# author-hidden-name/GAN-segmentation

Hardware: AMD Instinct MI355X
Metric: synthetic (image,mask) pairs/sec, FFHQ-1024 StyleGAN+decoder (higher is better)
Workload: dtype f32; 1 GPU; stylegan-ffhq 1024^2 synthesis + 2-class decoder, batch=8 per GPU, fp32 (BASELINE.json configs[1]); synthetic weights/latents/noise; (img u8, mask u8) resident on rank 0; global_batch=8, parallelism=dp1, gather=none, backend=none, graph=eager (GSA_GRAPH=0)

## Files before the change

### gan-segmentation_amd/csrc/gsa_api.cpp

```cpp
#include <hip/hip_runtime.h>

#include <cmath>
#include <cstdarg>
#include <cstdio>
#include <cstdlib>
#include <cstring>
#include <map>
#include <string>
#include <vector>

#include "../../include/gsa.h"
#include "gsa_kernels.h"
#include "gsa_pack.h"

using namespace gsa;

namespace {

constexpr int kMaxLevels = 12;
thread_local std::string g_create_error;

struct HostTensor {
    std::vector<float> data;
    std::vector<int64_t> dims;
// ... 780 lines not shown
                              uint8_t* img, float* const* feats, bool record_levels) {
    const int L = c->gc.latent_size, nlev = c->nlev;
    const double N = n;
    if (z) {
        if (int rc = run_mapping(c, s, n, z, c->lat[0])) return rc;
        const float* w = c->lat[0];
        Launch lp(c, s, "g.styles", 2.0 * N * L * c->style_cols, 4.0 * ((double)L * c->style_cols + N * c->style_cols));
        HIP_TRY(launch_styles(w, c->latent_avg, c->psi, c->style_wt, c->style_b, c->style_col_layer, c->styles, n, L, c->style_cols, s));
    } else {
        Launch lp(c, s, "g.styles", 2.0 * N * L * c->style_cols, 4.0 * ((double)L * c->style_cols + N * 2 * nlev * L + N * c->style_cols));
        HIP_TRY(launch_styles_dlatents(dl, c->latent_avg, c->psi, c->style_wt, c->style_b, c->style_tiles, c->style_num_tiles, c->styles, n, L,
                                       c->style_cols, 2 * nlev, s));
    }

    char layer[64];
    for (int l = 0; l < nlev; ++l) {
        const GenBlockDev& B = c->blk[l];
        const int R = B.R, C = B.C, Cin = B.Cin;
        const double px = N * R * R;
        for (int k = 0; k < 2; ++k) {
            const float* nz = noise[2 * l + k];
            if (!nz) return fail(c, GSA_ERR_INVALID, "noise plane %d is null", 2 * l + k);
            int prow = 0;
            if (k == 0) {
                PostParams pp{};
                pp.noise = nz; pp.nscale = B.nscale[0]; pp.nbias = B.nbias[0];
                pp.out = c->x1; pp.partials = c->partials; pp.H = R; pp.W = R; pp.C = C; pp.bf16 = c->bf16;
                if (!B.has_conv1) {
                    pp.src = c->constant; pp.src_per_sample = 0; pp.blur = nullptr;
                } else {
                    ConvParams cp = conv_base(c);
                    cp.src0 = c->x2[l - 1]; cp.aff0 = c->aff2[l - 1]; cp.C0 = Cin;
                    cp.Hs = R / 2; cp.Ws = R / 2; cp.H = R; cp.W = R;
                    cp.wpk = B.w1; cp.Cout = C; cp.out = c->t_raw;
                    if (B.is_deconv || R >= 16) {
                        snprintf(layer, sizeof layer, B.is_deconv ? "g.%d.deconv_1" : "g.%d.conv_1", R);
                        Launch lp(c, s, layer, 2.0 * px * C * Cin * (subpixel_uses_wino(cp) ? 2.25 : 4.0), 4.0 * (px / 4 * Cin + px * C), 2.0 * px * C * Cin * (B.is_deconv ? 4 : 9));
                        HIP_TRY(launch_subpixel(cp, EPI_RAW, false, n, s));
                    } else {
                        cp.up = 1;
                        snprintf(layer, sizeof layer, "g.%d.conv_1", R);
                        Launch lp(c, s, layer, 2.0 * px * C * Cin * 9, 4.0 * (px / 4 * Cin + px * C));
                        HIP_TRY(launch_conv3x3(cp, EPI_RAW, false, n, s));
                    }
                    pp.src = c->t_raw; pp.src_per_sample = 1; pp.blur = B.blur;
                }
                snprintf(layer, sizeof layer, "g.%d.post_1", R);
                if (post_fuses_finalize(pp)) {
                    FinalizeParams fp{};
                    fp.partials = c->partials; fp.prow = 0; fp.HW = R * R; fp.C = C; fp.acc = c->stat_acc; fp.tickets = c->stat_tickets;
                    fp.style = c->styles + B.style_off[0]; fp.style_stride = c->style_cols;
                    fp.gamma = B.gamma[0]; fp.beta = B.beta[0];
                    fp.aff = c->aff1;
                    fp.flags = c->map_ctl;
                    Launch lp(c, s, layer, 0.0, 4.0 * (2 * px * C + px));
                    HIP_TRY(launch_post_fin(pp, fp, n, s));
                    continue;
                }
                Launch lp(c, s, layer, 0.0, 4.0 * (2 * px * C + px));
#ifdef GSA_DBG_HOOKS
                if (!((c->dbg & 8) && R >= 512))
#endif
                HIP_TRY(launch_post(pp, n, s));
                prow = post_rows_used(pp);
            } else {
                ConvParams cp = conv_base(c);
                cp.src0 = c->x1; cp.aff0 = c->aff1; cp.C0 = C;
                cp.Hs = R; cp.Ws = R; cp.H = R; cp.W = R;
                cp.wpk = B.w2; cp.wino = B.w2u; cp.Cout = C; cp.out = c->x2[l];
                cp.noise = nz; cp.nscale = B.nscale[1]; cp.nbias = B.nbias[1]; cp.partials = c->partials;
                snprintf(layer, sizeof layer, "g.%d.conv_2", R);
                int rows = conv_stat_rows(R, R, C, n);
                cp.stat_rows_host = &rows;
                const bool fused_fin = conv_fuses_finalize(cp, EPI_SYNTH, false);
                const double products = conv_form_products(conv3x3_form(cp, EPI_SYNTH, false));
                if (fused_fin) {
                    cp.fin_style = c->styles + B.style_off[1]; cp.fin_style_stride = c->style_cols;
                    cp.fin_gamma = B.gamma[1]; cp.fin_beta = B.beta[1]; cp.fin_aff = c->aff2[l]; cp.fin_flags = c->map_ctl;
                }
                Launch lp(c, s, layer, 2.0 * px * C * C * products, 4.0 * (2 * px * C + px), 2.0 * px * C * C * 9);
                HIP_TRY(launch_conv3x3(cp, EPI_SYNTH, false, n, s));
                prow = rows;
                if (fused_fin) continue;
            }
            if (c->fault == 2 && l == 3 && k == 1) {
                c->fault = 0;
                return fail(c, GSA_ERR_HIP, "injected fault (gsa_debug_inject 2) between a statistics producer and its finalize");
            }
            FinalizeParams fp{};
            fp.partials = c->partials; fp.prow = prow; fp.HW = R * R; fp.C = C; fp.acc = c->stat_acc; fp.tickets = c->stat_tickets;
            fp.style = c->styles + B.style_off[k]; fp.style_stride = c->style_cols;
            fp.gamma = B.gamma[k]; fp.beta = B.beta[k];
            fp.aff = k == 0 ? c->aff1 : c->aff2[l];
            fp.flags = c->map_ctl;
            snprintf(layer, sizeof layer, "g.%d.finalize_%d", R, k + 1);
#ifdef GSA_DBG_HOOKS
            if ((c->dbg & 32) && ((k == 0 && R <= 32) || (k == 1 && R <= 8))) continue;
            if ((c->dbg & 64)) continue;
#endif
            Launch lp(c, s, layer, 0.0, 16.0 * N * prow * C);
            HIP_TRY(launch_finalize(fp, n, s));
        }
        if (record_levels) HIP_TRY(hipEventRecord(c->ev_level[l], s));
        if (feats && feats[l]) {
            snprintf(layer, sizeof layer, "g.%d.export", R);
            Launch lp(c, s, layer, 0.0, 8.0 * px * C);
            HIP_TRY(launch_export_nchw(c->x2[l], c->aff2[l], feats[l], n, R, R, C, c->bf16, s));
        }
    }
    if (rgb || img) {
        const int l = nlev - 1, R = c->blk[l].R, C = c->blk[l].C, nc = c->gc.channels;
// ... 354 lines not shown
```

### gan-segmentation_amd/csrc/gsa_dev.h

```cpp
#pragma once
#include "gsa_kernels.h"

#ifndef GSA_NO_XCD_REMAP
#define GSA_NO_XCD_REMAP 0
#endif

namespace gsa {

#ifdef GSA_STAMP
#define GSA_DBG_HOOKS 1
#endif
#ifdef GSA_STAMP
#define STAMP(i) do { __builtin_amdgcn_sched_barrier(0); asm volatile("s_memtime %0\n\ts_waitcnt lgkmcnt(0)" : "=s"(stamp_t[i]) :: "memory"); __builtin_amdgcn_sched_barrier(0); } while (0)
#define STAMP_DECL unsigned long long stamp_t[8] = {0, 0, 0, 0, 0, 0, 0, 0}
#define STAMP_FLUSH(nph) do { if (p.stamps && (threadIdx.x & 63) == 0) { for (int i_ = 0; i_ < (nph); ++i_) atomicAdd(&p.stamps[i_], stamp_t[i_ + 1] - stamp_t[i_]); atomicAdd(&p.stamps[15], 1ull); } } while (0)
#define TICK(var) do { __builtin_amdgcn_sched_barrier(0); asm volatile("s_memtime %0\n\ts_waitcnt lgkmcnt(0)" : "=s"(var) :: "memory"); __builtin_amdgcn_sched_barrier(0); } while (0)
#define TSUM(acc, a, b) acc += (b) - (a)
#define TFLUSH(idx, acc) do { if (p.stamps && (threadIdx.x & 63) == 0) atomicAdd(&p.stamps[idx], acc); } while (0)
#else
#define TICK(var) do {} while (0)
#define TSUM(acc, a, b) do {} while (0)
#define TFLUSH(idx, acc) do {} while (0)
#define STAMP(i) do {} while (0)
#define STAMP_DECL do {} while (0)
// ... 130 lines not shown

template <bool BF>
__device__ __forceinline__ f32x4 act_load4(const float* base, size_t idx) {
    if constexpr (BF) {
        const u32x2 r = *reinterpret_cast<const u32x2*>(reinterpret_cast<const unsigned short*>(base) + idx);
        return f32x4{bf16_lo(r[0]), bf16_hi(r[0]), bf16_lo(r[1]), bf16_hi(r[1])};
    } else {
        return *reinterpret_cast<const f32x4*>(base + idx);
    }
}

template <bool BF>
__device__ __forceinline__ void act_store4(float* base, size_t idx, const f32x4& v) {
    if constexpr (BF) {
        *reinterpret_cast<u32x2*>(reinterpret_cast<unsigned short*>(base) + idx) =
            u32x2{__builtin_bit_cast(unsigned, __builtin_convertvector(f32x2{v[0], v[1]}, bf16x2)),
                  __builtin_bit_cast(unsigned, __builtin_convertvector(f32x2{v[2], v[3]}, bf16x2))};
    } else {
        *reinterpret_cast<f32x4*>(base + idx) = v;
    }
}


__device__ __forceinline__ int xcd_block(int b, int nb) {
    return (nb & 7) == 0 && !GSA_NO_XCD_REMAP ? (b & 7) * (nb >> 3) + (b >> 3) : b;
}


}
```

### gan-segmentation_amd/csrc/gsa_kernels.h

```cpp
#pragma once
#include <hip/hip_runtime.h>
#include <stdint.h>
#include <stdlib.h>

#include <atomic>
#include <string>

namespace gsa {

struct Aff { float mean, A, B, pad; };

struct StatPart { unsigned long long s1, s2; };

constexpr double kStatScale1 = 268435456.0;

enum Epilogue { EPI_RAW = 0, EPI_SYNTH = 1, EPI_DEC = 2 };

struct ConvParams {
    int device;
    const float* src0; const Aff* aff0; int C0;
    const float* src1; int C1;
    int Hs, Ws;
    int up;
    int H, W;
    const float* wpk;
    const float* wino;
    int Cout;
    float* out;
    const float* noise; const float* nscale; const float* nbias;
    StatPart* partials; int prow;
    const float* bn_s; const float* bn_beta;
    const float* resid; int resid_up;
    const float* resid1; int res_c0;
    const float* wsc; const float* sc_bias; float* out_sc;
    int tiles_x, tiles_y, groups, total_tiles;
    int stats_direct;
    int* stat_rows_host;
    int w_resident;
    int group_minor;
    unsigned long long* stamps;
    int dbg;
    int prio;
    int bf16;
    const float* fin_style; int fin_style_stride; const float* fin_gamma; const float* fin_beta; Aff* fin_aff; unsigned* fin_flags;
    const float* zeros;
    const float* rgb_w; const float* rgb_b; uint8_t* rgb_img;
};

struct PostParams {
    const float* src;
    int src_per_sample;
    const float* blur;
    const float* noise; const float* nscale; const float* nbias;
    float* out; StatPart* partials; int prow;
    int H, W, C;
    int bf16;
    int row_groups;
};

struct FinalizeParams {
    const StatPart* partials; int prow; int HW; int C;
    StatPart* acc;
    unsigned* tickets;
    const float* style; int style_stride;
    const float* gamma; const float* beta;
    Aff* aff;
    unsigned* flags;
};

inline int env_int(const char* name, int dflt) {
    const char* v = getenv(name);
    return v ? atoi(v) : dflt;
}


enum class ConvForm { Wino43, WinoDma, WinoTwoTiles, WinoLean, Wino, KSplit, Bf16Lean, Direct };
ConvForm conv3x3_form(const ConvParams& p, int epi, bool shortcut);
hipError_t launch_conv3x3(const ConvParams& p, int epi, bool shortcut, int n, hipStream_t s);
inline bool conv_form_wino(ConvForm f) { return f <= ConvForm::Wino; }
inline double conv_form_products(ConvForm f) { return f == ConvForm::Wino43 ? 2.25 : conv_form_wino(f) ? 4 : 9; }
// ... 14 lines not shown
    int ct;
    SubPath path;
    bool wino;
    int kb;
    size_t lds;
    int wgs_per_group;
};
SubpixelPlan subpixel_plan(const ConvParams& p, bool shortcut, int n);
hipError_t launch_subpixel(const ConvParams& p, int epi, bool shortcut, int n, hipStream_t s);
bool subpixel_uses_wino(const ConvParams& p);
enum class PostKind { Dma, Packed, Rows, OneRow };
struct PostPlan { PostKind kind; int rpt, row_groups, blocks, rows_used; };
PostPlan post_plan(const PostParams& p);
hipError_t launch_post(const PostParams& p, int n, hipStream_t s);
int post_pk_mode();
bool post_dma_applies(const PostParams& p);
int post_dma_band(const PostParams& p);
int post_dma_blocks(const PostParams& p);
hipError_t launch_post_dma(const PostParams& p, int n, hipStream_t s);
hipError_t launch_post_pk(const PostParams& q, dim3 grid, size_t lds, hipStream_t s);
hipError_t launch_finalize(const FinalizeParams& p, int n, hipStream_t s);
bool conv_fuses_finalize(const ConvParams& p, int epi, bool shortcut);
bool post_fuses_finalize(const PostParams& p);
hipError_t launch_post_fin(const PostParams& p, const FinalizeParams& f, int n, hipStream_t s);
hipError_t launch_pixelnorm(const float* z, float* out, int n, int L, hipStream_t s);
constexpr int kMapSlices = 8;
bool mapping_fused(int L, int device);
hipError_t launch_mapping(const float* z, float* const* wt, float* const* b, unsigned long long* const* ll, float* out, unsigned* ctl,
                          int n, int L, int device, hipStream_t s, int drop_workgroups = 0);
hipError_t launch_dense(const float* x, const float* WT, const float* b, float* y, int n, int K, int J,
                        int lrelu, hipStream_t s);
hipError_t launch_styles(const float* w, const float* avg, const float* psi, const float* WT, const float* b,
                         const int* col_layer, float* styles, int n, int K, int J, hipStream_t s);
hipError_t launch_styles_dlatents(const float* dlatents, const float* avg, const float* psi, const float* WT, const float* b,
                                  const int4* tiles, int num_tiles, float* styles, int n, int K, int J, int NL, hipStream_t s);
hipError_t launch_torgb(const float* x, const Aff* aff, const float* w, const float* b, float* rgb,
                        uint8_t* img, int n, int H, int W, int C, int nc, int bf16, hipStream_t s);
hipError_t launch_torgb_down(const float* x, const Aff* aff, const float* w, const float* b, uint8_t* img, int n, int H, int W, int C,
                             int nc, int f, int bf16, hipStream_t s);
hipError_t launch_final_conv_down(const float* src0, int C0, const float* src1, int C1, const float* wpk, const float* bias, uint8_t* mask,
                                  int n, int H, int W, int ncls, int f, int bf16, hipStream_t s);
hipError_t launch_export_nchw(const float* x, const Aff* aff, float* out, int n, int H, int W, int C, int bf16, hipStream_t s);
hipError_t launch_import_nhwc(const float* in, float* out, int n, int H, int W, int C, int bf16, hipStream_t s);
hipError_t launch_final_conv(const float* src0, int C0, const float* src1, int C1, const float* wpk,
                             const float* bias, float* logits, uint8_t* mask, int n, int H, int W, int ncls, int bf16,
                             hipStream_t s);
// ... 45 lines not shown
```

### gan-segmentation_amd/csrc/gsa_kernels.hip

```cpp
#include "gsa_kernels.h"
#include "gsa_dev.h"

#include <cxxabi.h>

#include <cstdio>
#include <cstdlib>
#include <cstring>
#include <mutex>
#include <vector>

#ifndef GSA_MFMA_PRIO
#define GSA_MFMA_PRIO 2
#endif
#ifndef GSA_OPERAND_PIPELINE
#define GSA_OPERAND_PIPELINE 1
#endif
#ifndef GSA_NO_XCD_REMAP
#define GSA_NO_XCD_REMAP 0
#endif
#ifndef GSA_POST_OCC
#define GSA_POST_OCC 2
#endif
#ifndef GSA_WINO_SOA
#define GSA_WINO_SOA 0
// ... 628 lines not shown
        __syncthreads();
        if (has_aff && tn.n != n_aff) {
            write_aff();
            n_aff = tn.n;
            __syncthreads();
        }
#ifdef GSA_DBG_HOOKS
        if (!(p.dbg & 8))
#endif
        write_item(cb2, tpn, is_edge(tn));
        __syncthreads();
        tc = tn; w = w2; cb = cb2;
#pragma unroll
        for (int it = 0; it < AIT; ++it) tp[it] = tpn[it];
    }
    STAMP(4);
#ifdef GSA_STAMP
    asm volatile("s_waitcnt vmcnt(0)" ::: "memory");
#endif
    STAMP(5);
    STAMP_FLUSH(5);
}

__device__ __forceinline__ void finalize_one(const FinalizeParams& p, int n, int c, unsigned long long I1, unsigned long long I2);
template <int TH, int EPI, bool BF, int PS>
__global__ __launch_bounds__(256 * PS) void conv3x3_ksplit(ConvParams p) {
    constexpr int NTHR = 256 * PS, MT = (TH / 4) * (TH / 4), PW = TH / 4;
    constexpr int MTW = MT / PS;
    constexpr int LH = TH + 2, LW = TH + 2, NPX = LH * LW;
    constexpr int PX = BF ? 8 : 16, TS = BF ? 128 : 256, KQ = BF ? 2 : 4;
    constexpr int RS = LW * PX + (BF ? 4 : 8);
    constexpr int SEG = 9 * TS, IMG = LH * RS;
    constexpr int NB4 = 4 * SEG / 4, BIT = (NB4 + NTHR - 1) / NTHR;
    constexpr int QPT = PS == 1 ? 4 : 1;
    static_assert(PS == 1 || (PS == 2 && MT == 4 && 4 * NPX <= NTHR), "patch split: 8x8 tiles, one staged unit per thread");
    static_assert(NPX <= NTHR, "one staged pixel per thread and block");
    extern __shared__ __attribute__((aligned(16))) float smem[];
    float* sA = smem;
    float* sB = sA + 2 * 4 * IMG;
    f32x4* sAff = reinterpret_cast<f32x4*>(sB + 2 * 4 * SEG);
    f32x4* sP = sAff + 2 * 4 * 16;
    unsigned long long (*sfin)[16] = reinterpret_cast<unsigned long long (*)[16]>(sP + 4 * MT * 64);
    unsigned& sfin_cnt = *reinterpret_cast<unsigned*>(sfin + 2);
    if (EPI == EPI_SYNTH && p.fin_aff != nullptr && threadIdx.x < 33) {
        if (threadIdx.x < 32) sfin[threadIdx.x >> 4][threadIdx.x & 15] = 0ull; else sfin_cnt = 0u;
    }

// ... 1964 lines not shown
            }
        }
#pragma unroll
        for (int j = 0; j < 4; ++j) {
            atomicAdd(&sstat[c + j], I1[j]);
            atomicAdd(&sstat[p.C + c + j], I2[j]);
        }
    }
    __syncthreads();
    if ((int)gridDim.x > p.prow) {
        for (int i = threadIdx.x; i < p.C; i += 256) {
            StatPart* a = p.partials + ((size_t)n * p.prow + (blockIdx.x & (kDirectRows - 1))) * p.C + i;
            atomicAdd(&a->s1, sstat[i]);
            atomicAdd(&a->s2, sstat[p.C + i]);
        }
        return;
    }
    for (int i = threadIdx.x; i < p.C; i += 256) {
        StatPart sp; sp.s1 = sstat[i]; sp.s2 = sstat[p.C + i];
        p.partials[((size_t)n * p.prow + blockIdx.x) * p.C + i] = sp;
    }
}

__device__ __forceinline__ void finalize_one(const FinalizeParams& p, int n, int c, unsigned long long I1, unsigned long long I2) {
    const double inv_hw = 1.0 / (double)p.HW;
    const double m = (double)(long long)I1 * (1.0 / kStatScale1) * inv_hw;
    const double e2 = (double)(long long)I2 * (1.0 / stat_scale2(p.HW)) * inv_hw;
    double var = fma(-m, m, e2);
    {
        const long long s1 = (long long)I1;
        const bool near_wrap = (s1 < 0 ? -s1 : s1) >= (1ll << 61) || I2 >= (1ull << 61);
        if (p.flags && (near_wrap || var < -1e-6 * (e2 + m * m) - 1e-30)) atomicOr(p.flags, 1u);
    }
    if (!(var > 0.0)) var = 0.0;
    const float mean_f = (float)m, var_f = (float)var;
    const float inv = 1.0f / sqrtf(var_f + 1e-5f);
    const float gsc = p.gamma[c] * inv;
    const float* st = p.style + (size_t)n * p.style_stride;
    const float s1 = st[c] + 1.0f;
    Aff a;
    a.mean = mean_f;
    a.A = gsc * s1;
    a.B = fmaf(-mean_f, a.A, fmaf(p.beta[c], s1, st[p.C + c]));
    a.pad = 0.0f;
    p.aff[(size_t)n * p.C + c] = a;
}

__global__ __launch_bounds__(256) void finalize_kernel(FinalizeParams p, int rows_per_block) {
    __shared__ unsigned long long sh[2][256];
    __shared__ int is_last;
    const int n = blockIdx.y;
    const int cblk = p.C >= 64 ? 64 : p.C, nrg = 256 / cblk;
    const int cl = threadIdx.x % cblk, rg = threadIdx.x / cblk;
    const int c = blockIdx.x * 64 + cl;
    unsigned long long I1 = 0, I2 = 0;
    if (rg < nrg && c < p.C) {
        const int r0 = blockIdx.z * rows_per_block;
        const int r1 = min(p.prow, r0 + rows_per_block);
        const StatPart* base = p.partials + (size_t)n * p.prow * p.C + c;
#pragma unroll 16
        for (int r = r0 + rg; r < r1; r += nrg) {
            const StatPart sp = base[(size_t)r * p.C];
            I1 += sp.s1; I2 += sp.s2;
        }
        StatPart zero; zero.s1 = 0ull; zero.s2 = 0ull;
        StatPart* wbase = const_cast<StatPart*>(base);
        for (int r = r0 + rg; r < r1; r += nrg) wbase[(size_t)r * p.C] = zero;
    }
    sh[0][threadIdx.x] = I1; sh[1][threadIdx.x] = I2;
    __syncthreads();
// ... 933 lines not shown
    switch (conv3x3_form(p, epi, sc)) {
#if GSA_EXPERIMENTS
        case ConvForm::Wino43: return launch_wino43(p, epi, n, s);
        case ConvForm::WinoDma: return launch_wino_dma(p, epi, n, s);
        case ConvForm::WinoTwoTiles: return launch_wino_two_tiles(p, epi, n, s);
#endif
        case ConvForm::WinoLean: return launch_wino_lean(p, epi, n, s);
        case ConvForm::Wino: return launch_wino(p, epi, n, s);
        case ConvForm::KSplit: return launch_ksplit(p, epi, n, s);
        case ConvForm::Bf16Lean: return launch_bf16_lean(p, epi, n, s);
        case ConvForm::Direct: return launch_direct(p, epi, sc, n, s);
        default: return hipErrorInvalidValue;
    }
}

static bool fuse_finalize() {
    static const bool enabled = env_int("GSA_FUSEFIN", 1) != 0;
    return enabled;
}
bool conv_fuses_finalize(const ConvParams& p, int epi, bool sc) {
    return fuse_finalize() && epi == EPI_SYNTH && p.H <= 8 && conv3x3_form(p, epi, sc) == ConvForm::KSplit;
}

bool conv_fuses_torgb(const ConvParams& p, int epi, bool sc, int nc) {
    return conv3x3_form(p, epi, sc) == ConvForm::WinoLean && wino_lean_fuses_torgb(p, epi, nc);
}

bool subpixel_uses_wino(const ConvParams& p) {
    static const bool enabled = env_int("GSA_WINO22", 1) != 0;
    return enabled && !p.bf16;
}

SubpixelPlan subpixel_plan(const ConvParams& p, bool sc, int n) {
    static const bool res_enabled = env_int("GSA_SUBRES", 1) != 0;
    static const bool wst_enabled = env_int("GSA_SUBWST", 1) != 0;
    SubpixelPlan plan{};
    plan.wino = subpixel_uses_wino(p);
    const long tiles = (long)(p.H / 16) * (p.W / 16) * n;
    plan.ct = 16;
    for (int ct = plan.wino ? 32 : 64; ct > 16; ct /= 2)
        if (p.Cout % ct == 0 && tiles * (p.Cout / ct) >= 512) { plan.ct = ct; break; }
    const int ts = p.bf16 ? 128 : 256, nt = plan.ct / 16;
    const int rs = p.bf16 ? 10 * 8 + 4 : 10 * 16 + (plan.wino ? 4 : 8);
    if (res_enabled && plan.ct == p.Cout && plan.ct <= 32 && tiles >= 4096) {
        const int nblk = (p.C0 + p.C1) / 16;
        const size_t panel = sizeof(float) * ((size_t)nblk * nt * 16 * ts + (sc ? (size_t)nblk * nt * ts : 0));
// ... 106 lines not shown
    q.prow = plan.rows_used;
    q.row_groups = plan.row_groups;
    const dim3 grid(plan.blocks, n);
    const size_t lds = sizeof(unsigned long long) * 2 * p.C;
    const int dev = current_device();
    switch (plan.kind) {
        case PostKind::Dma: return launch_post_dma(q, n, s);
        case PostKind::Packed: return launch_post_pk(q, grid, lds + sizeof(float) * 9 * p.C, s);
        default: break;
    }
#define GSA_POST(BF) \
    if (plan.rpt == 8) return launch<post_rows_kernel<8, BF>>(dev, grid, dim3(256), lds, s, q); \
    if (plan.rpt == 4) return launch<post_rows_kernel<4, BF>>(dev, grid, dim3(256), lds, s, q); \
    if (plan.rpt == 2) return launch<post_rows_kernel<2, BF>>(dev, grid, dim3(256), lds, s, q); \
    return launch<post_kernel<BF>>(dev, grid, dim3(256), lds, s, q);
    if (p.bf16) { GSA_POST(true) }
    GSA_POST(false)
#undef GSA_POST
}

bool post_fuses_finalize(const PostParams& p) {
    return fuse_finalize() && p.H * p.W <= 1024 && p.C % 16 == 0 && p.W % 4 == 0;
}
hipError_t launch_post_fin(const PostParams& p, const FinalizeParams& f, int n, hipStream_t s) {
    if (!post_fuses_finalize(p)) return hipErrorInvalidValue;
    dim3 grid(p.C / 16, n);
    if (p.bf16) return launch<post_fin_kernel<true>>(current_device(), grid, dim3(256), 0, s, p, f);
    return launch<post_fin_kernel<false>>(current_device(), grid, dim3(256), 0, s, p, f);
}

hipError_t launch_finalize(const FinalizeParams& p, int n, hipStream_t s) {
    const int rpb = std::min(256, std::max(64, (p.prow + 15) / 16));
    const int zb = (p.prow + rpb - 1) / rpb;
    dim3 grid((p.C + 63) / 64, n, zb < 1 ? 1 : zb);
    return launch<finalize_kernel>(current_device(), grid, dim3(256), 0, s, p, rpb);
}

hipError_t launch_pixelnorm(const float* z, float* out, int n, int L, hipStream_t s) {
    return launch<pixelnorm_kernel>(current_device(), dim3(n), dim3(64), sizeof(float) * L, s, z, out, n, L);
}

hipError_t launch_dense(const float* x, const float* WT, const float* b, float* y, int n, int K, int J, int act, hipStream_t s) {
    if (K % 256 || J % 4) return hipErrorInvalidValue;
    const size_t lds = sizeof(float) * (256 * 16 + 16 * 256 + 256);
    return launch<dense_lds_kernel<false, 16, 256>>(current_device(), dim3((J + 15) / 16), dim3(256), lds, s, x, WT, b, y, n, K, J, act,
                  (const float*)nullptr, (const float*)nullptr, (const int*)nullptr);
// ... 112 lines not shown
```

### gan-segmentation_amd/csrc/gsa_post_lean.hip

```cpp
#include "gsa_kernels.h"
#include "gsa_dev.h"

#include <cstdlib>

namespace gsa {
namespace lean {

template <bool NT, bool BF>
__global__ __launch_bounds__(256, 2) void post_rows_pk(PostParams p) {
    constexpr int RPT = 4, ES = BF ? 2 : 4;
    extern __shared__ __attribute__((aligned(16))) unsigned long long sstat[];
    float* const sW = reinterpret_cast<float*>(sstat + 2 * p.C);
    const int n = blockIdx.y;
    const int C4 = p.C >> 2, W4 = p.W >> 2;
    const int NG = p.row_groups > 1 ? p.row_groups : 1;
    const int total = (p.H / (RPT * NG)) * W4 * C4;
    for (int i = threadIdx.x; i < 2 * p.C; i += 256) sstat[i] = 0ull;
    for (int i = threadIdx.x; i < 9 * p.C; i += 256) sW[(i % 9) * p.C + i / 9] = p.blur[i];
    __syncthreads();
    const int idx = xcd_block(blockIdx.x, gridDim.x) * 256 + threadIdx.x;
    if (idx < total) {
        const int cq = idx % C4, t = idx / C4;
        const int xq = t % W4;
        const int y0 = __builtin_amdgcn_readfirstlane((t / W4) * (RPT * NG));
        const int c = cq * 4, x0 = xq * 4;
        const char* const sb = reinterpret_cast<const char*>(p.src) + (size_t)n * p.H * p.W * p.C * ES;
        char* const ob = reinterpret_cast<char*>(p.out) + (size_t)n * p.H * p.W * p.C * ES;
        const char* const nzb = reinterpret_cast<const char*>(p.noise + (size_t)n * p.H * p.W);
        const volatile f32x4* wtap = reinterpret_cast<const volatile f32x4*>(sW + c);
// ... 59 lines not shown
                v01[q] = a; v23[q] = b;
                const f32x4 o = {a.x, a.y, b.x, b.y};
                char* dst = orow + xoff[1 + q];
                if constexpr (BF) act_store4<true>(reinterpret_cast<float*>(dst), 0, o);
                else if (NT) __builtin_nontemporal_store(o, reinterpret_cast<f32x4*>(dst));
                else *reinterpret_cast<f32x4*>(dst) = o;
            }
            const f32x2 s01 = (v01[0] + v01[1]) + (v01[2] + v01[3]);
            const f32x2 s23 = (v23[0] + v23[1]) + (v23[2] + v23[3]);
            const f32x2 q01 = (v01[0] * v01[0] + v01[1] * v01[1]) + (v01[2] * v01[2] + v01[3] * v01[3]);
            const f32x2 q23 = (v23[0] * v23[0] + v23[1] * v23[1]) + (v23[2] * v23[2] + v23[3] * v23[3]);
            I1[0] += to_fixed(s01.x, kStatScale1); I1[1] += to_fixed(s01.y, kStatScale1);
            I1[2] += to_fixed(s23.x, kStatScale1); I1[3] += to_fixed(s23.y, kStatScale1);
            I2[0] += to_fixed_sq(q01.x, s2); I2[1] += to_fixed_sq(q01.y, s2);
            I2[2] += to_fixed_sq(q23.x, s2); I2[3] += to_fixed_sq(q23.y, s2);
        }
#pragma unroll
        for (int j = 0; j < 4; ++j) {
            atomicAdd(&sstat[c + j], I1[j]);
            atomicAdd(&sstat[p.C + c + j], I2[j]);
        }
    }
    __syncthreads();
    if ((int)gridDim.x > p.prow) {
        for (int i = threadIdx.x; i < p.C; i += 256) {
            StatPart* a = p.partials + ((size_t)n * p.prow + (blockIdx.x & (kDirectRows - 1))) * p.C + i;
            atomicAdd(&a->s1, sstat[i]);
            atomicAdd(&a->s2, sstat[p.C + i]);
        }
        return;
    }
    for (int i = threadIdx.x; i < p.C; i += 256) {
        StatPart sp; sp.s1 = sstat[i]; sp.s2 = sstat[p.C + i];
        p.partials[((size_t)n * p.prow + blockIdx.x) * p.C + i] = sp;
    }
}


template <int C, bool OST>
__global__ __launch_bounds__(256, 1) void post_dma(PostParams p) {
    constexpr int CPP = C / 4, XT = 1024 / C, NPX = XT + 2, ICH = NPX * CPP, NCH = XT / 4, ROWF = (ICH + NCH) * 4, R = 8;
    static_assert(ICH > 256 && ICH + NCH <= 320, "five DMA instructions per ring row");
    extern __shared__ __attribute__((aligned(16))) float smem[];
    unsigned long long* const sstat = reinterpret_cast<unsigned long long*>(smem + 4 * R * ROWF + (OST ? 4 * 1024 : 0));
    const int tid = threadIdx.x, lane = tid & 63;
    const int wave = __builtin_amdgcn_readfirstlane(tid >> 6);
    float* const ring = smem + wave * R * ROWF;
    float* const orow_lds = smem + 4 * R * ROWF + wave * 1024;
    const int n = blockIdx.y, H = p.H, W = p.W, BH = p.row_groups;
    const int strips = W / XT, nbands = (H / BH) * strips;
    const int wb = __builtin_amdgcn_readfirstlane((int)xcd_block(blockIdx.x, gridDim.x) * 4 + wave);
    for (int i = tid; i < 2 * C; i += 256) sstat[i] = 0ull;
// ... 97 lines not shown
            }
            if constexpr (OST) {
                char* ocont = ob + (size_t)y * rowb + (unsigned)(x0 * C * 4) + lane * 16;
#pragma unroll
                for (int k = 0; k < 4; ++k) *reinterpret_cast<f32x4*>(ocont + k * 1024) = *reinterpret_cast<const f32x4*>(orow_lds + k * 256 + lane * 4);
            }
            const f32x2 s01 = (v01[0] + v01[1]) + (v01[2] + v01[3]);
            const f32x2 s23 = (v23[0] + v23[1]) + (v23[2] + v23[3]);
            const f32x2 q01 = (v01[0] * v01[0] + v01[1] * v01[1]) + (v01[2] * v01[2] + v01[3] * v01[3]);
            const f32x2 q23 = (v23[0] * v23[0] + v23[1] * v23[1]) + (v23[2] * v23[2] + v23[3] * v23[3]);
            I1[0] += to_fixed(s01.x, kStatScale1); I1[1] += to_fixed(s01.y, kStatScale1);
            I1[2] += to_fixed(s23.x, kStatScale1); I1[3] += to_fixed(s23.y, kStatScale1);
            I2[0] += to_fixed_sq(q01.x, s2); I2[1] += to_fixed_sq(q01.y, s2);
            I2[2] += to_fixed_sq(q23.x, s2); I2[3] += to_fixed_sq(q23.y, s2);
        }
        asm volatile("s_waitcnt vmcnt(0)" ::: "memory");
#pragma unroll
        for (int j = 0; j < 4; ++j) {
            atomicAdd(&sstat[c + j], I1[j]);
            atomicAdd(&sstat[C + c + j], I2[j]);
        }
    }
    __syncthreads();
    if ((int)gridDim.x > p.prow) {
        for (int i = threadIdx.x; i < C; i += 256) {
            StatPart* a = p.partials + ((size_t)n * p.prow + (blockIdx.x & (kDirectRows - 1))) * C + i;
            atomicAdd(&a->s1, sstat[i]);
            atomicAdd(&a->s2, sstat[C + i]);
        }
        return;
    }
    for (int i = threadIdx.x; i < C; i += 256) {
        StatPart sp; sp.s1 = sstat[i]; sp.s2 = sstat[C + i];
        p.partials[((size_t)n * p.prow + blockIdx.x) * C + i] = sp;
    }
}

}

int post_pk_mode() {
    static const int mode = env_int("GSA_POST_PK", 1);
    return mode;
}

int post_dma_band(const PostParams& p) {
    static const int forced = env_int("GSA_POST_DMA_BH", 0);
    if (forced >= 8 && forced % 4 == 0 && p.H % forced == 0) return forced;
    return (long)(p.H / 64) * (p.W / (1024 / p.C)) * 8 >= 2048 ? 64 : 32;
}

bool post_dma_applies(const PostParams& p) {
    static const bool on = env_int("GSA_POST_DMA", 1) != 0;
// ... 30 lines not shown
```

### gan-segmentation_amd/csrc/gsa_wino_lean.hip

```cpp
#include "gsa_kernels.h"
#include "gsa_dev.h"

#include <cstdio>
#include <cstdlib>
#include <type_traits>

namespace gsa {
namespace lean {

constexpr int LH = 18, LW = 18, RS = LW * 16 + 4;
constexpr int IMG = LH * RS;
constexpr int SEG = 16 * 256;
constexpr int NPIX = LH * LW;

struct Tile { int n, y0, x0; };

template <int EPI, bool AFF, bool RES, int NB, int GW, bool DB = true, int PF = 1, bool RGB = false>
__global__ __launch_bounds__(256 * GW, GW == 1 ? (DB ? 2 : 3) : 1) void conv3x3_wino_lean(ConvParams p) {
    static_assert(!RGB || (NB == 1 && GW == 1 && DB && AFF && EPI == EPI_DEC), "fused toRGB: the 16 -> 16 decoder kernel with an AdaIN source");
    static_assert(DB || (NB == 1 && GW == 1), "single-buffered form: one block, one group");
    static_assert(PF == 1 || (PF == 2 && DB), "two prefetch sets: the double-buffered form");
    constexpr int NTHR = 256 * GW, CIN = 16 * NB, COUT = 16 * GW;
    constexpr int NCH = (NPIX * 4 + NTHR - 1) / NTHR;
    constexpr bool kLastPartial = (NPIX * 4) % NTHR != 0;
    extern __shared__ __attribute__((aligned(16))) float smem[];
    float* const sA = smem;
    float* const sB = smem + (DB ? 2 : 1) * IMG;
    const int tid = threadIdx.x, lane = tid & 63;
    const int wave8 = __builtin_amdgcn_readfirstlane(tid >> 6);
    const int wave = wave8 & 3, gsel = wave8 >> 2;
    const int i16 = lane & 15, kq = lane >> 4, part = tid & 3;
    const int H = p.H, W = p.W;
    const int per = (p.total_tiles + (int)gridDim.x - 1) / (int)gridDim.x;
    const int w_begin = xcd_block(blockIdx.x, gridDim.x) * per;
    const int w_end = min(p.total_tiles, w_begin + per);
    if (w_begin >= w_end) return;
    const int items = (w_end - w_begin) * NB;

    {
        const f32x4* src = reinterpret_cast<const f32x4*>(p.wpk);
        f32x4 r[4];
#pragma unroll
        for (int h = 0; h < NB; ++h) {
#pragma unroll
            for (int j = 0; j < 4; ++j) r[j] = src[tid + NTHR * (4 * h + j)];
#pragma unroll
            for (int j = 0; j < 4; ++j) reinterpret_cast<f32x4*>(sB)[tid + NTHR * (4 * h + j)] = r[j];
        }
    }

    unsigned s_off[NCH], eflags = 0;
    int l_off[NCH];
#pragma unroll
    for (int k = 0; k < NCH; ++k) {
        const int pix = (tid + NTHR * k) >> 2;
        const bool real = pix < NPIX;
        const int ly = real ? pix / LW : 1, lx = real ? pix % LW : 1;
        s_off[k] = (unsigned)(((ly * W + lx) * CIN + part * 4) * 4);
        l_off[k] = real ? ly * RS + lx * 16 + part * 4 : -1;
        eflags |= (unsigned)((ly == 0 ? 1 : 0) | (ly == LH - 1 ? 2 : 0) | (lx == 0 ? 4 : 0) | (lx == LW - 1 ? 8 : 0)) << (4 * k);
// ... 253 lines not shown
            t3 = t2; e3c = e2c; cb3 = cb2;
            if (it + 3 < items) { next_item(t3, e3c, cb3); load_item(set_tag, t3, e3c, cb3); }
            TICK(k2);
            if (NB == 1 || cbc == 0) multiply(std::true_type{}, it & 1, 0);
            else multiply(std::false_type{}, it & 1, cbc);
            loads_landed(ra[PF - 1 - decltype(set_tag)::value], acc[15]);
            TICK(k3);
            if (cbc == NB - 1) {
                epilogue(tc);
                if (EPI == EPI_SYNTH && (!has_next || tr.n != tc.n)) flush_stats(tc.n);
            }
            TICK(k4);
            __syncthreads();
            TICK(k5);
            TSUM(sw, k0, k1); TSUM(sl, k1, k2); TSUM(sm, k2, k3); TSUM(se, k3, k4); TSUM(sb, k4, k5);
            tc = tr; ec = er; cbc = cbr; tr = t2; er = e2c; cbr = cb2; t2 = t3; e2c = e3c; cb2 = cb3;
        };
        for (int it = 0; it < items; it += 2) {
            body(S1{}, it);
            if (it + 1 < items) body(S0{}, it + 1);
        }
        TFLUSH(6, sw); TFLUSH(7, sl); TFLUSH(8, sm); TFLUSH(9, se); TFLUSH(10, sb);
        TFLUSH(12, (unsigned long long)items); TFLUSH(15, 1ull);
        return;
    }
    if (items > 1) { next_item(tr, er, cbr); load_item(S0{}, tr, er, cbr); }
    loads_landed(ra[0]);
    __syncthreads();
    if constexpr (DB) {
        for (int it = 0; it < items; ++it) {
            const bool has_next = it + 1 < items;
            TICK(k0);
            if (has_next) write_item(S0{}, tr, er, cbr, (it + 1) & 1);
            TICK(k1);
            if (cbc == NB - 1) epilogue_loads(tc);
            Tile t2 = tr; int e2c = er, cb2 = cbr;
            if (it + 2 < items) { next_item(t2, e2c, cb2); load_item(S0{}, t2, e2c, cb2); }
            TICK(k2);
            if (NB == 1 || cbc == 0) multiply(std::true_type{}, it & 1, 0);
            else multiply(std::false_type{}, it & 1, cbc);
            loads_landed(ra[0], acc[15]);
            TICK(k3);
            if constexpr (RGB) torgb(tc, it & 1);
            if (cbc == NB - 1) {
                epilogue(tc);
                if (EPI == EPI_SYNTH && (!has_next || tr.n != tc.n)) flush_stats(tc.n);
// ... 3 lines not shown
            TICK(k5);
            TSUM(sw, k0, k1); TSUM(sl, k1, k2); TSUM(sm, k2, k3); TSUM(se, k3, k4); TSUM(sb, k4, k5);
            tc = tr; ec = er; cbc = cbr; tr = t2; er = e2c; cbr = cb2;
        }
        TFLUSH(6, sw); TFLUSH(7, sl); TFLUSH(8, sm); TFLUSH(9, se); TFLUSH(10, sb);
        TFLUSH(12, (unsigned long long)items); TFLUSH(15, 1ull);
    } else {
        for (int it = 0; it < items; ++it) {
            const bool has_next = it + 1 < items;
            transform(0);
            __syncthreads();
            if (has_next) write_item(S0{}, tr, er, 0, 0);
            epilogue_loads(tc);
            Tile t2 = tr; int e2c = er, cb2 = 0;
            if (it + 2 < items) { next_item(t2, e2c, cb2); load_item(S0{}, t2, e2c, cb2); }
            mfmas(std::true_type{}, 0);
            loads_landed(ra[0], acc[15]);
            epilogue(tc);
            if (EPI == EPI_SYNTH && (!has_next || tr.n != tc.n)) flush_stats(tc.n);
            __syncthreads();
            tc = tr; ec = er; tr = t2; er = e2c;
        }
    }
}

__device__ unsigned g_cu_tickets[4096];
__device__ __forceinline__ void antiphase_start(int cycles64, float* lds_word) {
    if (cycles64 <= 0) return;
    if (threadIdx.x == 0) {
        unsigned hw, xcc;
        asm volatile("s_getreg_b32 %0, hwreg(HW_REG_HW_ID)" : "=s"(hw));
        asm volatile("s_getreg_b32 %0, hwreg(HW_REG_XCC_ID)" : "=s"(xcc));
        const unsigned cu = ((xcc & 15u) << 8) | (((hw >> 13) & 7u) << 5) | (((hw >> 12) & 1u) << 4) | ((hw >> 8) & 15u);
        *reinterpret_cast<unsigned*>(lds_word) = atomicAdd(&g_cu_tickets[cu & 4095u], 1u);
    }
    __syncthreads();
    const unsigned ticket = *reinterpret_cast<volatile unsigned*>(lds_word);
    __syncthreads();
    if (ticket & 1u)
        for (int i = 0; i < cycles64; i += 16) __builtin_amdgcn_s_sleep(16);
}

template <int EPI, bool AFF, int NT, int IL, bool PAIR>
__device__ __forceinline__ void wino_stream_body(const ConvParams& p) {
    static_assert(!PAIR || (NT == 1 && IL == 0), "paired form: one group per wave quad, phased memory instructions");
    constexpr int NTHR = PAIR ? 512 : 256;
// ... 326 lines not shown
        TICK(k1);
        if (cbc == nblk - 1) epilogue_loads(tc);
        Tile t2 = tr; int e2c = er, cb2 = cbr;
        if (it + 2 < items) { next_item(t2, e2c, cb2); if (!IL) load_item(t2, e2c, cb2); }
        TICK(k2);
        auto vm0 = [&]() { if (IL == 1 && has_next) dma_weights(cbr, (it + 1) & 1); };
        auto vm1 = [&]() { if (IL == 1 && it + 2 < items) load_item(t2, e2c, cb2); };
        if (cbc == 0) multiply(std::true_type{}, it & 1, vm0, vm1);
        else multiply(std::false_type{}, it & 1, vm0, vm1);
        vmem_drained(accs[NT - 1][15]);
        TICK(k3);
        if (cbc == nblk - 1) {
            epilogue(tc);
            if (EPI == EPI_SYNTH && (!has_next || tr.n != tc.n)) flush_stats(tc.n);
        }
        TICK(k4);
        __syncthreads();
        TICK(k5);
        TSUM(sw, k0, k1); TSUM(sl, k1, k2); TSUM(sm, k2, k3); TSUM(se, k3, k4); TSUM(sb, k4, k5);
        tc = tr; ec = er; cbc = cbr; tr = t2; er = e2c; cbr = cb2;
    }
    TFLUSH(6, sw); TFLUSH(7, sl); TFLUSH(8, sm); TFLUSH(9, se); TFLUSH(10, sb);
    TFLUSH(12, (unsigned long long)items); TFLUSH(15, 1ull);
}

template <int EPI, bool AFF, int NT = 1, int IL = 0>
__global__ __launch_bounds__(256, NT == 1 ? 2 : 1) void conv3x3_wino_stream(ConvParams p) {
    wino_stream_body<EPI, AFF, NT, IL, false>(p);
}

template <int EPI, bool AFF>
__global__ __launch_bounds__(512, 1) void conv3x3_wino_stream_pair(ConvParams p) {
    wino_stream_body<EPI, AFF, 1, 0, true>(p);
}

template <int EPI, bool AFF, bool RES, int NB, int GW, bool DB = true, int PF = 1, bool RGB = false>
hipError_t launch_t(const ConvParams& p, int n, hipStream_t s) {
    const size_t lds = sizeof(float) * ((DB ? 2 : 1) * IMG + GW * NB * SEG);
    const int cus = device_cus(p.device);
    ConvParams q = p;
    q.wpk = p.wino;
    q.tiles_x = p.W / 16;
    q.tiles_y = p.H / 16;
    q.groups = 1;
    q.total_tiles = q.tiles_x * q.tiles_y * n;
    if (EPI == EPI_SYNTH) {
// ... 60 lines not shown
    q.group_minor = PAIR ? 0 : stagger;
#else
    q.group_minor = 0;
#endif
    q.total_tiles = q.tiles_x * q.tiles_y * n;
    if (EPI == EPI_SYNTH) {
        q.stats_direct = 1;
        q.prow = kDirectRows;
        if (p.stat_rows_host) *p.stat_rows_host = q.prow;
    }
    const int slots = std::max(1, cus * (NP == 1 ? 2 : 1) / q.groups);
    const int gx = std::min(q.total_tiles, slots);
    if constexpr (PAIR) return launch<conv3x3_wino_stream_pair<EPI, AFF>>(p.device, dim3(gx, q.groups), dim3(512), lds, s, q);
    else return launch<conv3x3_wino_stream<EPI, AFF, NT, IL>>(p.device, dim3(gx, q.groups), dim3(256), lds, s, q);
}

}
using namespace lean;

bool wino_lean_applies(const ConvParams& p, int epi) {
    static const int enabled = env_int("GSA_WINO_LEAN", 7);
    if (p.H != p.W || p.H % 16) return false;
    if ((enabled & 4) && p.C0 >= 64 && p.C0 <= 512 && p.resid == nullptr && p.H >= 16)
        return epi == EPI_SYNTH ? (p.partials != nullptr && p.noise != nullptr && p.fin_aff == nullptr) : epi == EPI_DEC;
    const bool shape = (p.C0 == 16 && p.Cout == 16 && (enabled & 1)) || (p.C0 == 32 && p.Cout == 32 && (enabled & 2));
    if (!shape || p.H < 32) return false;
    if (epi == EPI_SYNTH) return p.partials != nullptr && p.noise != nullptr && p.fin_aff == nullptr && p.resid == nullptr;
    if (epi != EPI_DEC) return false;
    if (p.resid != nullptr && (p.resid_up != 1 || p.resid1 != nullptr)) return false;
    return true;
}

bool wino_lean_fuses_torgb(const ConvParams& p, int epi, int nc) {
    static const bool enabled = env_int("GSA_FUSE_RGB", 1) != 0;
    return enabled && nc == 3 && epi == EPI_DEC && p.C0 == 16 && p.Cout == 16 && p.aff0 != nullptr && p.resid == nullptr && !p.bf16 &&
           wino_lean_applies(p, epi) && !single_buffered();
}

bool wino_stream_paired(const ConvParams& p, int n) {
    static const int mode = env_int("GSA_WINO_PAIR", 1);
    if (mode <= 0 || p.C0 < 64 || p.Cout % 32) return false;
    if (mode == 2) return true;
    return (long)(p.W / 16) * (p.H / 16) * n * (p.Cout / 32) >= device_cus(p.device);
}

bool stream_pairs(const ConvParams& p, int n) {
#if GSA_EXPERIMENTS
    static const int on = env_int("GSA_WINO_NT2", 0);
    if (!on || p.Cout % 32) return false;
    const long wgs = (long)(p.W / 16) * (p.H / 16) * n * (p.Cout / 32);
// ... 48 lines not shown
```

Baseline: 1416 pairs/s.

## Finalize instance-norm statistics in the last producer block via tickets

Result: no change. 1417 pairs/s (median of 3 runs) (+0.0%).

```diff
diff --git a/gan-segmentation_amd/csrc/gsa_api.cpp b/gan-segmentation_amd/csrc/gsa_api.cpp
--- a/gan-segmentation_amd/csrc/gsa_api.cpp
+++ b/gan-segmentation_amd/csrc/gsa_api.cpp
@@ -826,6 +826,7 @@
             const float* nz = noise[2 * l + k];
             if (!nz) return fail(c, GSA_ERR_INVALID, "noise plane %d is null", 2 * l + k);
             int prow = 0;
+            bool prod_fin = false;
             if (k == 0) {
                 PostParams pp{};
                 pp.noise = nz; pp.nscale = B.nscale[0]; pp.nbias = B.nbias[0];
@@ -861,6 +862,12 @@
                     HIP_TRY(launch_post_fin(pp, fp, n, s));
                     continue;
                 }
+                prod_fin = post_finalizes_in_producer(pp);
+                if (prod_fin) {
+                    pp.fin_style = c->styles + B.style_off[0]; pp.fin_style_stride = c->style_cols;
+                    pp.fin_gamma = B.gamma[0]; pp.fin_beta = B.beta[0]; pp.fin_aff = c->aff1; pp.fin_flags = c->map_ctl;
+                    pp.fin_tickets = c->stat_tickets;
+                }
                 Launch lp(c, s, layer, 0.0, 4.0 * (2 * px * C + px));
 #ifdef GSA_DBG_HOOKS
                 if (!((c->dbg & 8) && R >= 512))
@@ -878,10 +885,12 @@
                 cp.stat_rows_host = &rows;
                 const bool fused_fin = conv_fuses_finalize(cp, EPI_SYNTH, false);
                 const double products = conv_form_products(conv3x3_form(cp, EPI_SYNTH, false));
-                if (fused_fin) {
+                prod_fin = !fused_fin && conv_finalizes_in_producer(cp, EPI_SYNTH, false);
+                if (fused_fin || prod_fin) {
                     cp.fin_style = c->styles + B.style_off[1]; cp.fin_style_stride = c->style_cols;
                     cp.fin_gamma = B.gamma[1]; cp.fin_beta = B.beta[1]; cp.fin_aff = c->aff2[l]; cp.fin_flags = c->map_ctl;
                 }
+                if (prod_fin) cp.fin_tickets = c->stat_tickets;
                 Launch lp(c, s, layer, 2.0 * px * C * C * products, 4.0 * (2 * px * C + px), 2.0 * px * C * C * 9);
                 HIP_TRY(launch_conv3x3(cp, EPI_SYNTH, false, n, s));
                 prow = rows;
@@ -891,6 +900,7 @@
                 c->fault = 0;
                 return fail(c, GSA_ERR_HIP, "injected fault (gsa_debug_inject 2) between a statistics producer and its finalize");
             }
+            if (prod_fin) continue;
             FinalizeParams fp{};
             fp.partials = c->partials; fp.prow = prow; fp.HW = R * R; fp.C = C; fp.acc = c->stat_acc; fp.tickets = c->stat_tickets;
             fp.style = c->styles + B.style_off[k]; fp.style_stride = c->style_cols;
diff --git a/gan-segmentation_amd/csrc/gsa_dev.h b/gan-segmentation_amd/csrc/gsa_dev.h
--- a/gan-segmentation_amd/csrc/gsa_dev.h
+++ b/gan-segmentation_amd/csrc/gsa_dev.h
@@ -176,6 +176,77 @@
 }
 
 
+__device__ __forceinline__ void finalize_one(const FinalizeParams& p, int n, int c, unsigned long long I1, unsigned long long I2) {
+    const double inv_hw = 1.0 / (double)p.HW;
+    const double m = (double)(long long)I1 * (1.0 / kStatScale1) * inv_hw;
+    const double e2 = (double)(long long)I2 * (1.0 / stat_scale2(p.HW)) * inv_hw;
+    double var = fma(-m, m, e2);
+    {
+        const long long s1 = (long long)I1;
+        const bool near_wrap = (s1 < 0 ? -s1 : s1) >= (1ll << 61) || I2 >= (1ull << 61);
+        if (p.flags && (near_wrap || var < -1e-6 * (e2 + m * m) - 1e-30)) atomicOr(p.flags, 1u);
+    }
+    if (!(var > 0.0)) var = 0.0;
+    const float mean_f = (float)m, var_f = (float)var;
+    const float inv = 1.0f / sqrtf(var_f + 1e-5f);
+    const float gsc = p.gamma[c] * inv;
+    const float* st = p.style + (size_t)n * p.style_stride;
+    const float s1 = st[c] + 1.0f;
+    Aff a;
+    a.mean = mean_f;
+    a.A = gsc * s1;
+    a.B = fmaf(-mean_f, a.A, fmaf(p.beta[c], s1, st[p.C + c]));
+    a.pad = 0.0f;
+    p.aff[(size_t)n * p.C + c] = a;
+}
+
+template <int NTHR, class Count>
+__device__ __forceinline__ void producer_finalize(const FinalizeParams& f, unsigned* tickets, int n0, int n1, Count count, unsigned expected,
+                                                  unsigned long long* acc, unsigned* flag) {
+    const int tid = threadIdx.x;
+    asm volatile("s_waitcnt vmcnt(0)" ::: "memory");
+    __syncthreads();
+    StatPart* const rows = const_cast<StatPart*>(f.partials);
+    for (int n = n0; n <= n1; ++n) {
+        if (tid == 0) {
+            const unsigned k = count(n);
+            const unsigned t = __hip_atomic_fetch_add(tickets + n, k, __ATOMIC_RELAXED, __HIP_MEMORY_SCOPE_AGENT);
+            const bool last = k != 0 && t + k == expected;
+            if (last) {
+                __hip_atomic_store(tickets + n, 0u, __ATOMIC_RELAXED, __HIP_MEMORY_SCOPE_AGENT);
+                __builtin_amdgcn_fence(__ATOMIC_ACQUIRE, "agent");
+                asm volatile("s_waitcnt vmcnt(0)" ::: "memory");
+            }
+            *flag = last ? 1u : 0u;
+        }
+        for (int i = tid; i < 2 * f.C; i += NTHR) acc[i] = 0ull;
+        __syncthreads();
+        const bool last = *reinterpret_cast<volatile unsigned*>(flag) != 0;
+        if (last) {
+            for (int cb = 0; cb < f.C; cb += NTHR) {
+                const int cw = min(NTHR, f.C - cb), nrg = NTHR / cw;
+                const int c = cb + tid % cw, rg = tid / cw;
+                if (rg < nrg) {
+                    StatPart* base = rows + (size_t)n * f.prow * f.C + c;
+                    unsigned long long I1 = 0ull, I2 = 0ull;
+#pragma unroll 16
+                    for (int r = rg; r < f.prow; r += nrg) {
+                        const StatPart sp = base[(size_t)r * f.C];
+                        I1 += sp.s1; I2 += sp.s2;
+                    }
+                    StatPart zero; zero.s1 = 0ull; zero.s2 = 0ull;
+                    for (int r = rg; r < f.prow; r += nrg) base[(size_t)r * f.C] = zero;
+                    atomicAdd(&acc[c], I1);
+                    atomicAdd(&acc[f.C + c], I2);
+                }
+            }
+            __syncthreads();
+            for (int c = tid; c < f.C; c += NTHR) finalize_one(f, n, c, acc[c], acc[f.C + c]);
+        }
+        __syncthreads();
+    }
+}
+
 __device__ __forceinline__ int xcd_block(int b, int nb) {
     return (nb & 7) == 0 && !GSA_NO_XCD_REMAP ? (b & 7) * (nb >> 3) + (b >> 3) : b;
 }
diff --git a/gan-segmentation_amd/csrc/gsa_kernels.h b/gan-segmentation_amd/csrc/gsa_kernels.h
--- a/gan-segmentation_amd/csrc/gsa_kernels.h
+++ b/gan-segmentation_amd/csrc/gsa_kernels.h
@@ -45,6 +45,7 @@
     const float* fin_style; int fin_style_stride; const float* fin_gamma; const float* fin_beta; Aff* fin_aff; unsigned* fin_flags;
     const float* zeros;
     const float* rgb_w; const float* rgb_b; uint8_t* rgb_img;
+    unsigned* fin_tickets;
 };
 
 struct PostParams {
@@ -56,6 +57,8 @@
     int H, W, C;
     int bf16;
     int row_groups;
+    const float* fin_style; int fin_style_stride; const float* fin_gamma; const float* fin_beta; Aff* fin_aff; unsigned* fin_flags;
+    unsigned* fin_tickets;
 };
 
 struct FinalizeParams {
@@ -116,6 +119,9 @@
 hipError_t launch_finalize(const FinalizeParams& p, int n, hipStream_t s);
 bool conv_fuses_finalize(const ConvParams& p, int epi, bool shortcut);
 bool post_fuses_finalize(const PostParams& p);
+int fin_producer_mode();
+bool conv_finalizes_in_producer(const ConvParams& p, int epi, bool shortcut);
+bool post_finalizes_in_producer(const PostParams& p);
 hipError_t launch_post_fin(const PostParams& p, const FinalizeParams& f, int n, hipStream_t s);
 hipError_t launch_pixelnorm(const float* z, float* out, int n, int L, hipStream_t s);
 constexpr int kMapSlices = 8;
diff --git a/gan-segmentation_amd/csrc/gsa_kernels.hip b/gan-segmentation_amd/csrc/gsa_kernels.hip
--- a/gan-segmentation_amd/csrc/gsa_kernels.hip
+++ b/gan-segmentation_amd/csrc/gsa_kernels.hip
@@ -674,7 +674,6 @@
     STAMP_FLUSH(5);
 }
 
-__device__ __forceinline__ void finalize_one(const FinalizeParams& p, int n, int c, unsigned long long I1, unsigned long long I2);
 template <int TH, int EPI, bool BF, int PS>
 __global__ __launch_bounds__(256 * PS) void conv3x3_ksplit(ConvParams p) {
     constexpr int NTHR = 256 * PS, MT = (TH / 4) * (TH / 4), PW = TH / 4;
@@ -2685,30 +2684,6 @@
     }
 }
 
-__device__ __forceinline__ void finalize_one(const FinalizeParams& p, int n, int c, unsigned long long I1, unsigned long long I2) {
-    const double inv_hw = 1.0 / (double)p.HW;
-    const double m = (double)(long long)I1 * (1.0 / kStatScale1) * inv_hw;
-    const double e2 = (double)(long long)I2 * (1.0 / stat_scale2(p.HW)) * inv_hw;
-    double var = fma(-m, m, e2);
-    {
-        const long long s1 = (long long)I1;
-        const bool near_wrap = (s1 < 0 ? -s1 : s1) >= (1ll << 61) || I2 >= (1ull << 61);
-        if (p.flags && (near_wrap || var < -1e-6 * (e2 + m * m) - 1e-30)) atomicOr(p.flags, 1u);
-    }
-    if (!(var > 0.0)) var = 0.0;
-    const float mean_f = (float)m, var_f = (float)var;
-    const float inv = 1.0f / sqrtf(var_f + 1e-5f);
-    const float gsc = p.gamma[c] * inv;
-    const float* st = p.style + (size_t)n * p.style_stride;
-    const float s1 = st[c] + 1.0f;
-    Aff a;
-    a.mean = mean_f;
-    a.A = gsc * s1;
-    a.B = fmaf(-mean_f, a.A, fmaf(p.beta[c], s1, st[p.C + c]));
-    a.pad = 0.0f;
-    p.aff[(size_t)n * p.C + c] = a;
-}
-
 __global__ __launch_bounds__(256) void finalize_kernel(FinalizeParams p, int rows_per_block) {
     __shared__ unsigned long long sh[2][256];
     __shared__ int is_last;
@@ -3688,6 +3663,18 @@
     return fuse_finalize() && epi == EPI_SYNTH && p.H <= 8 && conv3x3_form(p, epi, sc) == ConvForm::KSplit;
 }
 
+int fin_producer_mode() {
+    static const int mode = env_int("GSA_FIN_PRODUCER", 1);
+    return mode;
+}
+static bool fin_producer_plane(int H) {
+    const int mode = fin_producer_mode();
+    return mode == 2 || (mode == 1 && H >= 64);
+}
+bool conv_finalizes_in_producer(const ConvParams& p, int epi, bool sc) {
+    return fin_producer_plane(p.H) && epi == EPI_SYNTH && !conv_fuses_finalize(p, epi, sc) && conv3x3_form(p, epi, sc) == ConvForm::WinoLean;
+}
+
 bool conv_fuses_torgb(const ConvParams& p, int epi, bool sc, int nc) {
     return conv3x3_form(p, epi, sc) == ConvForm::WinoLean && wino_lean_fuses_torgb(p, epi, nc);
 }
@@ -3840,6 +3827,12 @@
 bool post_fuses_finalize(const PostParams& p) {
     return fuse_finalize() && p.H * p.W <= 1024 && p.C % 16 == 0 && p.W % 4 == 0;
 }
+bool post_finalizes_in_producer(const PostParams& p) {
+    if (!fin_producer_plane(p.H) || post_fuses_finalize(p) || p.W % 4 || p.C % 4) return false;
+    const PostPlan plan = post_plan(p);
+    if (plan.rows_used > kDirectRows) return false;
+    return plan.kind == PostKind::Dma || (plan.kind == PostKind::Packed && fin_producer_mode() == 2);
+}
 hipError_t launch_post_fin(const PostParams& p, const FinalizeParams& f, int n, hipStream_t s) {
     if (!post_fuses_finalize(p)) return hipErrorInvalidValue;
     dim3 grid(p.C / 16, n);
diff --git a/gan-segmentation_amd/csrc/gsa_post_lean.hip b/gan-segmentation_amd/csrc/gsa_post_lean.hip
--- a/gan-segmentation_amd/csrc/gsa_post_lean.hip
+++ b/gan-segmentation_amd/csrc/gsa_post_lean.hip
@@ -5,6 +5,13 @@
 
 namespace gsa {
 namespace lean {
+
+__device__ __forceinline__ void post_finalize(const PostParams& p, int n, unsigned long long* acc, unsigned* flag) {
+    FinalizeParams f;
+    f.partials = p.partials; f.prow = p.prow; f.HW = p.H * p.W; f.C = p.C; f.acc = nullptr; f.tickets = nullptr;
+    f.style = p.fin_style; f.style_stride = p.fin_style_stride; f.gamma = p.fin_gamma; f.beta = p.fin_beta; f.aff = p.fin_aff; f.flags = p.fin_flags;
+    producer_finalize<256>(f, p.fin_tickets, n, n, [](int) { return 1u; }, gridDim.x, acc, flag);
+}
 
 template <bool NT, bool BF>
 __global__ __launch_bounds__(256, 2) void post_rows_pk(PostParams p) {
@@ -110,12 +117,13 @@
         }
     }
     __syncthreads();
-    if ((int)gridDim.x > p.prow) {
+    if ((int)gridDim.x > p.prow || p.fin_aff != nullptr) {
         for (int i = threadIdx.x; i < p.C; i += 256) {
             StatPart* a = p.partials + ((size_t)n * p.prow + (blockIdx.x & (kDirectRows - 1))) * p.C + i;
             atomicAdd(&a->s1, sstat[i]);
             atomicAdd(&a->s2, sstat[p.C + i]);
         }
+        if (p.fin_aff != nullptr) post_finalize(p, n, sstat, reinterpret_cast<unsigned*>(sW));
         return;
     }
     for (int i = threadIdx.x; i < p.C; i += 256) {
@@ -259,12 +267,13 @@
         }
     }
     __syncthreads();
-    if ((int)gridDim.x > p.prow) {
+    if ((int)gridDim.x > p.prow || p.fin_aff != nullptr) {
         for (int i = threadIdx.x; i < C; i += 256) {
             StatPart* a = p.partials + ((size_t)n * p.prow + (blockIdx.x & (kDirectRows - 1))) * C + i;
             atomicAdd(&a->s1, sstat[i]);
             atomicAdd(&a->s2, sstat[C + i]);
         }
+        if (p.fin_aff != nullptr) post_finalize(p, n, sstat, reinterpret_cast<unsigned*>(smem));
         return;
     }
     for (int i = threadIdx.x; i < C; i += 256) {
diff --git a/gan-segmentation_amd/csrc/gsa_wino_lean.hip b/gan-segmentation_amd/csrc/gsa_wino_lean.hip
--- a/gan-segmentation_amd/csrc/gsa_wino_lean.hip
+++ b/gan-segmentation_amd/csrc/gsa_wino_lean.hip
@@ -14,6 +14,18 @@
 constexpr int NPIX = LH * LW;
 
 struct Tile { int n, y0, x0; };
+
+template <int NTHR>
+__device__ __forceinline__ void wino_finalize(const ConvParams& p, int w_begin, int w_end, float* smem) {
+    FinalizeParams f;
+    f.partials = p.partials; f.prow = p.prow; f.HW = p.H * p.W; f.C = p.Cout; f.acc = nullptr; f.tickets = nullptr;
+    f.style = p.fin_style; f.style_stride = p.fin_style_stride; f.gamma = p.fin_gamma; f.beta = p.fin_beta; f.aff = p.fin_aff; f.flags = p.fin_flags;
+    const int T = p.tiles_x * p.tiles_y;
+    unsigned long long* acc = reinterpret_cast<unsigned long long*>(smem);
+    producer_finalize<NTHR>(f, p.fin_tickets, w_begin / T, (w_end - 1) / T,
+                            [&](int n) { return (unsigned)(min(w_end, (n + 1) * T) - max(w_begin, n * T)); },
+                            (unsigned)T * gridDim.y, acc, reinterpret_cast<unsigned*>(acc + 2 * p.Cout));
+}
 
 template <int EPI, bool AFF, bool RES, int NB, int GW, bool DB = true, int PF = 1, bool RGB = false>
 __global__ __launch_bounds__(256 * GW, GW == 1 ? (DB ? 2 : 3) : 1) void conv3x3_wino_lean(ConvParams p) {
@@ -36,6 +48,11 @@
     const int w_end = min(p.total_tiles, w_begin + per);
     if (w_begin >= w_end) return;
     const int items = (w_end - w_begin) * NB;
+    auto finish = [&]() {
+        if constexpr (EPI == EPI_SYNTH) {
+            if (p.fin_tickets != nullptr) wino_finalize<NTHR>(p, w_begin, w_end, smem);
+        }
+    };
 
     {
         const f32x4* src = reinterpret_cast<const f32x4*>(p.wpk);
@@ -335,6 +352,7 @@
         }
         TFLUSH(6, sw); TFLUSH(7, sl); TFLUSH(8, sm); TFLUSH(9, se); TFLUSH(10, sb);
         TFLUSH(12, (unsigned long long)items); TFLUSH(15, 1ull);
+        finish();
         return;
     }
     if (items > 1) { next_item(tr, er, cbr); load_item(S0{}, tr, er, cbr); }
@@ -384,6 +402,7 @@
             tc = tr; ec = er; tr = t2; er = e2c;
         }
     }
+    finish();
 }
 
 __device__ unsigned g_cu_tickets[4096];
@@ -756,6 +775,9 @@
     }
     TFLUSH(6, sw); TFLUSH(7, sl); TFLUSH(8, sm); TFLUSH(9, se); TFLUSH(10, sb);
     TFLUSH(12, (unsigned long long)items); TFLUSH(15, 1ull);
+    if constexpr (EPI == EPI_SYNTH) {
+        if (p.fin_tickets != nullptr) wino_finalize<NTHR>(p, w_begin, w_end, smem);
+    }
 }
 
 template <int EPI, bool AFF, int NT = 1, int IL = 0>
@@ -862,10 +884,10 @@
     static const int enabled = env_int("GSA_WINO_LEAN", 7);
     if (p.H != p.W || p.H % 16) return false;
     if ((enabled & 4) && p.C0 >= 64 && p.C0 <= 512 && p.resid == nullptr && p.H >= 16)
-        return epi == EPI_SYNTH ? (p.partials != nullptr && p.noise != nullptr && p.fin_aff == nullptr) : epi == EPI_DEC;
+        return epi == EPI_SYNTH ? (p.partials != nullptr && p.noise != nullptr && (p.fin_aff == nullptr || p.fin_tickets != nullptr)) : epi == EPI_DEC;
     const bool shape = (p.C0 == 16 && p.Cout == 16 && (enabled & 1)) || (p.C0 == 32 && p.Cout == 32 && (enabled & 2));
     if (!shape || p.H < 32) return false;
-    if (epi == EPI_SYNTH) return p.partials != nullptr && p.noise != nullptr && p.fin_aff == nullptr && p.resid == nullptr;
+    if (epi == EPI_SYNTH) return p.partials != nullptr && p.noise != nullptr && (p.fin_aff == nullptr || p.fin_tickets != nullptr) && p.resid == nullptr;
     if (epi != EPI_DEC) return false;
     if (p.resid != nullptr && (p.resid_up != 1 || p.resid1 != nullptr)) return false;
     return true;
```
